# kotaro-kinoshita/yomitoku

Hardware: AMD Instinct MI355X
Metric: pages/sec (DocumentAnalyzer @1600x1200, lite model set) (higher is better)
Workload: dtype f32 held as two scaled fp16 planes per operand on the MFMA pipe: 3 x v_mfma_f32_32x32x16_f16 per product tile (products to 2^-21, below the fp32 accumulation's own rounding), fp32 accumulate, fp32 activations in HBM; attention, LayerNorm, the fused greedy step and every grid-starved launch exact fp3

## Files before the change

### yomitoku_amd/csrc/ymk_api.cpp

```cpp
#include "../../include/ymk.h"
#include "ymk_common.h"
#include "ymk_decstep.h"
#include "ymk_det.h"
#include "ymk_entry.h"
#include "ymk_seq.h"

struct ymk_model {
  ymk::Model* impl = nullptr;
  int device = 0;
};

#include <dlfcn.h>
namespace {
struct Roctx {
  int (*push)(const char*) = nullptr;
  int (*pop)() = nullptr;
  Roctx() {
    const char* on = std::getenv("YMK_ROCTX");
    if (on == nullptr || on[0] == '\0' || on[0] == '0') return;
    for (const char* name : {"librocprofiler-sdk-roctx.so", "libroctx64.so"}) {
      if (void* h = dlopen(name, RTLD_NOW | RTLD_GLOBAL)) {
        push = reinterpret_cast<int (*)(const char*)>(dlsym(h, "roctxRangePushA"));
        pop = reinterpret_cast<int (*)()>(dlsym(h, "roctxRangePop"));
        if (push && pop) return;
// ... 26 lines not shown
    return 1;                                       \
  }                                                 \
  catch (...) {                                     \
    ymk::set_error("unknown C++ exception");        \
    return 2;                                       \
  }

extern "C" {

int ymk_version(void) { return 100; }

const char* ymk_last_error(void) { return ymk::last_error().c_str(); }

int ymk_device_count(void) {
  int n = 0;
  if (hipGetDeviceCount(&n) != hipSuccess) return -1;
  return n;
}

ymk_model* ymk_model_create(const char* kind, int device) {
  try {
    YMK_CHECK(kind != nullptr, "kind is null");
    YMK_HIP(hipSetDevice(device));
    std::string k(kind);
    ymk::Model* impl = nullptr;
    if (k == "dbnet") impl = ymk::create_dbnet();
    else if (k == "parseq") impl = ymk::create_parseq();
    else if (k == "rtdetr") impl = ymk::create_rtdetr();
    else throw ymk::Error("unknown model kind: " + k);
    auto* m = new ymk_model();
    m->impl = impl;
    m->device = device;
    return m;
  } catch (const std::exception& e) {
    ymk::set_error(e.what());
    return nullptr;
  }
}

void ymk_model_destroy(ymk_model* m) {
  if (!m) return;
  (void)hipSetDevice(m->device);
  delete m->impl;
  delete m;
}

int ymk_model_set_param(ymk_model* m, const char* key, double value) {
  YMK_API_BEGIN
  YMK_CHECK(m && key, "null argument");
  const std::string k(key);
  if (k == "workspace_reuse") {
    YMK_CHECK(value == 0.0 || value == 1.0 || value == -1.0, "workspace_reuse must be 0 or 1 (-1: follow the process-wide default)");
    YMK_CHECK(!ymk::in_forward(), "workspace_reuse cannot change inside a forward");
  }
  m->impl->params[key] = value;
  if (m->impl->finalized && (k == "conv_split" || k == "conv_split_encoder")) {
    YMK_HIP(hipSetDevice(m->device));
    m->impl->prebuild_split();
  }
  YMK_API_END
}

int ymk_model_set_tensor(ymk_model* m, const char* name, const float* host_data, int ndim, const int64_t* dims) {
  YMK_API_BEGIN
  YMK_CHECK(m && name && host_data && (ndim == 0 || dims), "null argument");
  YMK_CHECK(!m->impl->finalized, "model already finalized");
  m->impl->ws.put(name, host_data, ndim, dims);
  YMK_API_END
}

int ymk_model_finalize(ymk_model* m) {
  YMK_API_BEGIN
  RoctxRange roctx_range("ymk_model_finalize");
  YMK_CHECK(m, "null model");
  YMK_HIP(hipSetDevice(m->device));
  m->impl->finalize();
  m->impl->prebuild_split();
  if (!ymk::debug_hazard_no_finalize_sync()) YMK_HIP(hipDeviceSynchronize());
  YMK_API_END
}

int ymk_model_reserve(ymk_model* m, int n, int h, int w, void* stream) {
  YMK_API_BEGIN
  RoctxRange roctx_range("ymk_model_reserve");
  YMK_CHECK(m && m->impl, "null argument");
  YMK_HIP(hipSetDevice(m->device));
  m->impl->reserve(n, h, w, (hipStream_t)stream);
  YMK_API_END
}

int64_t ymk_model_weight_bytes(const ymk_model* m) { return m ? (int64_t)m->impl->pool.bytes() : -1; }
int64_t ymk_model_workspace_bytes(const ymk_model* m) { return m ? (int64_t)m->impl->arena.capacity() : -1; }

int ymk_dbnet_forward(ymk_model* m, const float* x_dev, int n, int h, int w, float* prob_dev, void* stream) {
  YMK_API_BEGIN
  RoctxRange roctx_range("ymk_dbnet_forward");
  YMK_CHECK(m && x_dev && prob_dev, "null argument");
  YMK_HIP(hipSetDevice(m->device));
  ymk::dbnet_forward(m->impl, x_dev, n, h, w, prob_dev, (hipStream_t)stream);
  YMK_API_END
}

int ymk_parseq_dims(ymk_model* m, int* num_steps, int* num_classes) {
  YMK_API_BEGIN
  YMK_CHECK(m && num_steps && num_classes, "null argument");
  ymk::parseq_dims(m->impl, num_steps, num_classes);
  YMK_API_END
}

int ymk_parseq_forward(ymk_model* m, const float* x_dev, int b, int w, float* logits_dev, int* out_len, int* ar_steps,
                       void* stream) {
  YMK_API_BEGIN
  RoctxRange roctx_range("ymk_parseq_forward");
  YMK_CHECK(m && x_dev && logits_dev && out_len && ar_steps, "null argument");
  YMK_HIP(hipSetDevice(m->device));
  ymk::parseq_forward(m->impl, x_dev, b, w, logits_dev, out_len, ar_steps, (hipStream_t)stream);
  YMK_API_END
}

int ymk_parseq_forward_groups(ymk_model* m, const float* const* x_dev, const int* b, const int* w, int n_groups,
                              float* logits_dev, int* out_len, int* ar_steps, void* stream) {
  YMK_API_BEGIN
  RoctxRange roctx_range("ymk_parseq_forward_groups");
  YMK_CHECK(m && x_dev && b && w && logits_dev && out_len && ar_steps, "null argument");
  YMK_HIP(hipSetDevice(m->device));
  ymk::parseq_forward_groups(m->impl, x_dev, b, w, n_groups, logits_dev, out_len, ar_steps, (hipStream_t)stream);
  YMK_API_END
}

int ymk_parseq_token_stats(const float* logits_dev, int rows, int num_classes, int* ids_dev, float* probs_dev,
                           void* stream) {
  YMK_API_BEGIN
  RoctxRange roctx_range("ymk_parseq_token_stats");
  YMK_CHECK(logits_dev && ids_dev && probs_dev, "null argument");
  ymk::row_maxprob((hipStream_t)stream, logits_dev, rows, num_classes, ids_dev, probs_dev);
  YMK_API_END
}

int ymk_rtdetr_forward(ymk_model* m, const float* x_dev, int b, int h, int w, float* logits_dev, float* boxes_dev,
                       void* stream) {
  YMK_API_BEGIN
  RoctxRange roctx_range("ymk_rtdetr_forward");
  YMK_CHECK(m && x_dev && logits_dev && boxes_dev, "null argument");
  YMK_HIP(hipSetDevice(m->device));
  ymk::rtdetr_forward(m->impl, x_dev, b, h, w, logits_dev, boxes_dev, (hipStream_t)stream);
  YMK_API_END
}

int ymk_debug_option(const char* key, int value) {
  YMK_API_BEGIN
  YMK_CHECK(key != nullptr, "null key");
  const std::string k(key);
  YMK_CHECK(ymk::conv_debug_option(k, value) || ymk::parseq_debug_option(k, value) || ymk::decstep_debug_option(k, value) ||
                ymk::conv_split_debug_option(k, value) || ymk::runtime_debug_option(k, value),
            "unknown debug option: " + k);
  YMK_API_END
}

int ymk_stat(const char* key, int64_t* value) {
  YMK_API_BEGIN
  YMK_CHECK(key != nullptr && value != nullptr, "null argument");
  long long v = 0;
  YMK_CHECK(ymk::conv_split_stat(std::string(key), &v) || ymk::runtime_stat(std::string(key), &v) || ymk::parseq_stat(std::string(key), &v), std::string("unknown counter: ") + key);
  *value = v;
  YMK_API_END
}

int ymk_amax_check_counters(int64_t* out4) {
  YMK_API_BEGIN
  YMK_CHECK(out4 != nullptr, "null argument");
  long long v[4];
  ymk::amax_check_counters(v);
  for (int i = 0; i < 4; ++i) out4[i] = v[i];
  YMK_API_END
}

int ymk_prof_begin(void) {
  YMK_API_BEGIN
  ymk::prof_begin();
  YMK_API_END
}

int ymk_prof_end(double* conv_ms, double* conv_flop, int64_t* conv_launches) {
  YMK_API_BEGIN
  YMK_CHECK(conv_ms && conv_flop && conv_launches, "null argument");
  ymk::prof_end(conv_ms, conv_flop, conv_launches);
  YMK_API_END
}

int ymk_prof_bytes(double* conv_bytes) {
  YMK_API_BEGIN
  YMK_CHECK(conv_bytes, "null argument");
  *conv_bytes = ymk::prof_bytes();
  YMK_API_END
}

int ymk_prof_launch_table(double* ms, double* flop, double* bytes, double* mfma_products, int64_t capacity, int64_t* count) {
  YMK_API_BEGIN
  YMK_CHECK(count != nullptr && capacity >= 0 && (capacity == 0 || (ms && flop && bytes && mfma_products)), "null argument");
  *count = ymk::prof_launch_table(ms, flop, bytes, mfma_products, capacity);
  YMK_API_END
}

int ymk_op_plan_workspace(int64_t n, const int64_t* sizes, const int64_t* release_pos, int64_t* offsets_out, int64_t* peak_out,
                          int64_t* live_bound_out) {
  YMK_API_BEGIN
  YMK_CHECK(n >= 0 && (n == 0 || (sizes && offsets_out)), "plan_workspace: bad argument");
  std::vector<size_t> sz((size_t)n), off((size_t)n);
  for (int64_t k = 0; k < n; ++k) {
    YMK_CHECK(sizes[k] >= 0, "plan_workspace: negative size");
    sz[(size_t)k] = (size_t)sizes[k];
  }
  size_t peak = 0, live = 0;
  ymk::plan_workspace((size_t)n, sz.data(), release_pos, off.data(), &peak, &live);
  for (int64_t k = 0; k < n; ++k) offsets_out[k] = (int64_t)off[(size_t)k];
  if (peak_out) *peak_out = (int64_t)peak;
  if (live_bound_out) *live_bound_out = (int64_t)live;
  YMK_API_END
}

int ymk_op_conv2d(const float* x_dev, int n, int h, int w, int c, const float* w_host_oihw, int cout, int cin, int kh,
                  int kw, const float* scale_host, const float* bias_host, const float* res_dev, int stride, int pad,
                  int dil, int act, int tap4, float* y_dev, void* stream) {
  YMK_API_BEGIN
  using namespace ymk;
  DevicePool pool;
  ConvW cw;
  cw.cout = cout;
  cw.cin = tap4 ? 4 : cin;
  cw.kh = kh;
  cw.kw = kw;
  cw.mode = tap4 ? 1 : 0;
  std::vector<float> panel;
  pack_conv_weight(w_host_oihw, cout, cin, kh, kw, tap4 != 0, panel, cw.kpad, cw.ctiles);
  cw.w = pool.upload(panel);
  if (scale_host) cw.scale = pool.upload(scale_host, cout);
  if (bias_host) cw.bias = pool.upload(bias_host, cout);
  Tensor in{const_cast<float*>(x_dev), n, h, w, c, c};
  const int oh = conv_out_dim(h, kh, stride, pad, dil), ow = conv_out_dim(w, kw, stride, pad, dil);
  Tensor out{y_dev, n, oh, ow, cout, cout};
  Tensor res{const_cast<float*>(res_dev), n, oh, ow, cout, cout};
  ConvArgs a;
  a.stride = stride;
  a.pad = pad;
  a.dil = dil;
  a.act = act;
  a.res = res_dev ? &res : nullptr;
  SplitCtxOwner split_ctx;
  ConvSplitScope scope(-1, split_ctx.get(), 0);
  conv2d((hipStream_t)stream, in, cw, a, out);
  YMK_HIP(hipStreamSynchronize((hipStream_t)stream));
  YMK_API_END
}

static ymk::ConvW op_conv_weight(ymk::DevicePool& pool, const float* w_host_oihw, int cout, int cin, int kh, int kw, bool tap4,
                                 const float* scale_host, const float* bias_host) {
  using namespace ymk;
  ConvW cw;
  cw.cout = cout;
  cw.cin = tap4 ? 4 : cin;
  cw.kh = kh;
  cw.kw = kw;
  cw.mode = tap4 ? 1 : 0;
  std::vector<float> panel;
  pack_conv_weight(w_host_oihw, cout, cin, kh, kw, tap4, panel, cw.kpad, cw.ctiles);
  cw.w = pool.upload(panel);
  std::vector<float> scale, bias;
  if (scale_host) scale.assign(scale_host, scale_host + cout);
  if (bias_host) bias.assign(bias_host, bias_host + cout);
  if (scale_host) cw.scale = pool.upload(scale);
  if (bias_host) cw.bias = pool.upload(bias);
  plane_bound(cw, w_host_oihw, (size_t)cin * kh * kw, scale, bias);
  return cw;
}

int ymk_op_conv2d_view(const float* x_dev, int n, int h, int w, int c, int in_ld, const float* w_host_oihw, int cout, int kh, int kw,
                       int tap4, const float* scale_host, const float* bias_host, const float* res_dev, int res_ld, int res_post,
                       int stride_h, int stride_w, int pad, int dil, int act, const int* row_group_dev, const int* group_open_dev,
                       const unsigned* amax_in_dev, unsigned* amax_out_dev, float* y_dev, int out_ld, void* stream) {
  YMK_API_BEGIN
  using namespace ymk;
  YMK_CHECK(x_dev && w_host_oihw && y_dev, "null argument");
  YMK_CHECK(n > 0 && h > 0 && w > 0 && c > 0 && in_ld > 0 && cout > 0 && kh > 0 && kw > 0 && res_ld >= 0 && out_ld > 0 &&
                stride_h > 0 && stride_w > 0 && pad >= 0 && dil > 0,
            "conv2d_view: sizes, strides and leading dimensions are positive (res_ld may be 0)");
  hipStream_t s = (hipStream_t)stream;
  DevicePool pool;
  const ConvW cw = op_conv_weight(pool, w_host_oihw, cout, c, kh, kw, tap4 != 0, scale_host, bias_host);
  SplitCtxOwner split_ctx;
  ConvSplitScope scope(-1, split_ctx.get(), 0);
  if (row_group_dev || group_open_dev) {
    YMK_CHECK(kh == 1 && kw == 1 && stride_h == 1 && stride_w == 1 && pad == 0 && !res_post && !tap4,
              "conv2d_view: a row predicate comes with a plain linear layer");
    gemm(s, x_dev, n * h * w, c, in_ld, cw, act, res_dev, res_ld, y_dev, out_ld, row_group_dev, group_open_dev, EPI_STORE, amax_in_dev,
         amax_out_dev);
  } else {
    Tensor in{const_cast<float*>(x_dev), n, h, w, c, in_ld};
    const int oh = conv_out_dim(h, kh, stride_h, pad, dil), ow = conv_out_dim(w, kw, stride_w, pad, dil);
    Tensor out{y_dev, n, oh, ow, cout, out_ld};
    Tensor res{const_cast<float*>(res_dev), n, oh, ow, cout, res_ld};
    ConvArgs a;
    a.stride = stride_h;
    a.stride_w = stride_w;
    a.pad = pad;
    a.dil = dil;
    a.act = act;
    a.res = res_dev ? &res : nullptr;
    a.res_post = res_post != 0;
    a.amax_in = amax_in_dev;
    a.amax_out = amax_out_dev;
    conv2d(s, in, cw, a, out);
  }
  YMK_HIP(hipStreamSynchronize(s));
  YMK_API_END
}

// ... 475 lines not shown
```

### yomitoku_amd/csrc/ymk_seq.h

```cpp
#pragma once
#include "ymk_common.h"

namespace ymk {

void layernorm(hipStream_t s, const float* x, int ldx, int in_rows_mod, const float* g, const float* b, float eps,
               float* y, int ldy, int M, int D);
void add_pos_embed(hipStream_t s, float* x, const float* pos, int B, int gh, int gw, int full_gw, int D);

struct SeqTab {
  const int *qoff = nullptr, *qlen = nullptr, *koff = nullptr, *klen = nullptr;
};

void flash_attention(hipStream_t s, const float* q, const float* k, const float* v, float* o, int B, int H, int Lq, int Lk,
                     int hd, int ldq, int ldk, int ldv, int ldo, long bsq, long bsk, long bsv, long bso, float scale,
                     const SeqTab* tab = nullptr, const unsigned* amax_q = nullptr, const unsigned* amax_k = nullptr,
                     const unsigned* amax_v = nullptr);
void small_attention(hipStream_t s, const float* q, const float* k, const float* v, float* o, int B, int H, int Lq, int Lk,
                     int hd, int ldq, int ldk, int ldv, int ldo, long bsq, long bsk, long bsv, long bso, float scale,
                     const unsigned char* mask_qk, int ld_mask, const unsigned char* kpm, int ld_kpm,
                     const SeqTab* tab = nullptr);
void nar_cross_attention(hipStream_t s, const float* q, const float* k, const float* v, float* o, int B, int H, int Lq, int Lk,
                         int hd, int ldq, int ldk, int ldv, int ldo, long bsk, long bsv, long bso, float scale,
                         const SeqTab* tab = nullptr);
void init_decode(hipStream_t s, int* tok, int ld_tok, int* state, int bos_id, int pad_id, int B);

void ctx_embed_ln(hipStream_t s, const int* tok, int ld_tok, int pos0, int npos, const float* emb, const float* posq,
                  const float* g, const float* be, float eps, float* out, int out_rows, int D, int B);
void greedy_step(hipStream_t s, const float* logits, long ld_b, int C, int step, int num_steps, int* tok, int* raw,
                 int ld_tok, int* state, int eos_id, int rep_on, int period_max, int min_run_p1, int min_repeats,
                 int* not_done, const int* prev_not_done, int* arrived, int* host_flag, int B, const int* gid = nullptr,
                 int* gopen = nullptr, int ng = 1, int partials = 0);
void publish_open(hipStream_t s, const int* not_done, const int* prev_not_done, int* host_flag);
void refine_prep(hipStream_t s, const int* raw, int ld_tok, int S, int bos_id, int eos_id, int* tok2, unsigned char* kpm,
                 int B, const int* gid = nullptr, const int* gsteps = nullptr);
void row_argmax(hipStream_t s, const float* logits, int rows, int C, int* out);
void rep_cut(hipStream_t s, float* logits, long ld_b, int C, int S, const int* state, int eos_id, int B);
void row_maxprob(hipStream_t s, const float* logits, int rows, int C, int* ids, float* probs);
void tile_rows(hipStream_t s, const float* src, int rows, int D, float* dst, int B);
void fill_i32(hipStream_t s, int* p, int v, size_t n);

}
```

### yomitoku_amd/csrc/ymk_seq.hip

```cpp
#include "ymk_common.h"
#include "ymk_f16_planes.h"
#include "ymk_seq.h"

namespace ymk {


__device__ __forceinline__ float wave_sum(float v) {
#pragma unroll
  for (int o = 32; o > 0; o >>= 1) v += __shfl_xor(v, o, 64);
  return v;
}
__device__ __forceinline__ float wave_max(float v) {
#pragma unroll
  for (int o = 32; o > 0; o >>= 1) v = fmaxf(v, __shfl_xor(v, o, 64));
  return v;
}

__global__ void k_layernorm(const float* __restrict__ x, int ldx, int in_rows_mod, const float* __restrict__ g,
                            const float* __restrict__ b, float eps, float* __restrict__ y, int ldy, int M, int D) {
  const int row = blockIdx.x * (blockDim.x >> 6) + (threadIdx.x >> 6);
  const int lane = threadIdx.x & 63;
  if (row >= M) return;
  const float* xr = x + (size_t)(in_rows_mod > 0 ? row % in_rows_mod : row) * ldx;
  float4 v[4];
  const int nv = D >> 2;
  float s = 0.f;
#pragma unroll
  for (int i = 0; i < 4; ++i) {
    const int c = lane + 64 * i;
    if (c < nv) {
      v[i] = *reinterpret_cast<const float4*>(xr + c * 4);
      s += (v[i].x + v[i].y) + (v[i].z + v[i].w);
    }
  }
  const float mean = wave_sum(s) / (float)D;
  float q = 0.f;
#pragma unroll
  for (int i = 0; i < 4; ++i) {
    const int c = lane + 64 * i;
    if (c < nv) {
      const float a = v[i].x - mean, bb = v[i].y - mean, cc = v[i].z - mean, d = v[i].w - mean;
      q += (a * a + bb * bb) + (cc * cc + d * d);
    }
  }
  const float rstd = 1.f / sqrtf(wave_sum(q) / (float)D + eps);
#pragma unroll
  for (int i = 0; i < 4; ++i) {
    const int c = lane + 64 * i;
    if (c < nv) {
      const float4 gg = *reinterpret_cast<const float4*>(g + c * 4);
      const float4 be = *reinterpret_cast<const float4*>(b + c * 4);
      float4 o;
      o.x = (v[i].x - mean) * rstd * gg.x + be.x;
      o.y = (v[i].y - mean) * rstd * gg.y + be.y;
      o.z = (v[i].z - mean) * rstd * gg.z + be.z;
      o.w = (v[i].w - mean) * rstd * gg.w + be.w;
      *reinterpret_cast<float4*>(y + (size_t)row * ldy + c * 4) = o;
    }
  }
}
void layernorm(hipStream_t s, const float* x, int ldx, int in_rows_mod, const float* g, const float* b, float eps,
               float* y, int ldy, int M, int D) {
  YMK_CHECK(D % 4 == 0 && D <= 1024, "layernorm: D must be a multiple of 4, <= 1024");
  if (M == 0) return;
  hipLaunchKernelGGL(k_layernorm, dim3((M + 3) / 4), dim3(256), 0, s, x, ldx, in_rows_mod, g, b, eps, y, ldy, M, D);
  YMK_HIP(hipGetLastError());
}

__global__ void k_add_pos(float* __restrict__ x, const float* __restrict__ pos, int gh, int gw, int full_gw, int D4,
                          size_t total) {
  for (size_t i = (size_t)blockIdx.x * blockDim.x + threadIdx.x; i < total; i += (size_t)gridDim.x * blockDim.x) {
    const int c4 = (int)(i % D4);
    const size_t tok = i / D4;
    const int cc = (int)(tok % gw);
    const int rr = (int)((tok / gw) % gh);
    float4 v = reinterpret_cast<float4*>(x)[i];
    const float4 p = reinterpret_cast<const float4*>(pos)[(size_t)(rr * full_gw + cc) * D4 + c4];
    v.x += p.x; v.y += p.y; v.z += p.z; v.w += p.w;
    reinterpret_cast<float4*>(x)[i] = v;
  }
}
void add_pos_embed(hipStream_t s, float* x, const float* pos, int B, int gh, int gw, int full_gw, int D) {
  const size_t total = (size_t)B * gh * gw * (D / 4);
  size_t g = (total + 255) / 256;
  if (g > 4096) g = 4096;
  hipLaunchKernelGGL(k_add_pos, dim3((int)g), dim3(256), 0, s, x, pos, gh, gw, full_gw, D / 4, total);
  YMK_HIP(hipGetLastError());
}

struct AttnP {
  const float *q, *k, *v;
  float* o;
  int ldq, ldk, ldv, ldo;
  long bsq, bsk, bsv, bso;
  int Lq, Lk, H;
  float scale;
  const int *qoff, *qlen, *koff, *klen;
  const unsigned *amax_q, *amax_k, *amax_v;
};

template <int HD, int HDR = HD>
__global__ __launch_bounds__(256, 1) void k_flash_attn(AttnP p) {
  constexpr int KT = 64;
  constexpr int LDH = HD + 4;
  constexpr int NKC = HDR / 8;
  constexpr int NDC = HD / 32;
  constexpr int LPT = (KT * HDR / 4) / 256;
  static_assert(HD % 32 == 0 && HDR % 8 == 0 && HDR <= HD && (KT * HDR / 4) % 256 == 0, "head dim");
  __shared__ __attribute__((aligned(16))) float lds[2 * 2 * KT * LDH];

  const int t = threadIdx.x, wv = t >> 6, lane = t & 63, li = lane & 31, lh = lane >> 5;
  const int b = blockIdx.z, h = blockIdx.y;
  const int q0 = blockIdx.x * 128 + wv * 32;
  const float* qb = p.q + (size_t)b * p.bsq + h * HDR;
  const float* kb = p.k + (size_t)b * p.bsk + h * HDR;
  const float* vb = p.v + (size_t)b * p.bsv + h * HDR;
  float* ob = p.o + (size_t)b * p.bso + h * HDR;
  int Lq = p.Lq, Lk = p.Lk;
  if (p.koff) {
    const size_t r = (size_t)p.koff[b];
    kb = p.k + r * p.ldk + h * HDR;
    vb = p.v + r * p.ldv + h * HDR;
    Lk = p.klen[b];
  }
  if (p.qoff) {
    const size_t r = (size_t)p.qoff[b];
    qb = p.q + r * p.ldq + h * HDR;
    ob = p.o + r * p.ldo + h * HDR;
    Lq = p.qlen[b];
  }
  if ((int)blockIdx.x * 128 >= Lq) return;

  f32x4 qf[NKC];
  {
    const int qi = min(q0 + li, Lq - 1);
    const float* qr = qb + (size_t)qi * p.ldq;
#pragma unroll
    for (int kc = 0; kc < NKC; ++kc) {
      qf[kc] = *reinterpret_cast<const f32x4*>(qr + kc * 8 + lh * 4);
      qf[kc] *= p.scale;
    }
  }

  f32x16 oacc[NDC];
#pragma unroll
  for (int dc = 0; dc < NDC; ++dc)
#pragma unroll
    for (int r = 0; r < 16; ++r) oacc[dc][r] = 0.f;
  float m_run = -INFINITY, l_run = 0.f;

  f32x4 rk[LPT], rv[LPT];
  auto load_kv = [&](int k0) {
// ... 173 lines not shown
      const int idx = t + 256 * i;
      const int row = idx / (HDR / 4), c4 = idx - row * (HDR / 4);
      *reinterpret_cast<f32x4*>(Ks + row * LDH + c4 * 4) = rk[i];
      *reinterpret_cast<f32x4*>(Vs + row * LDH + c4 * 4) = rv[i];
    }
  };

  const int ntiles = (Lk + KT - 1) / KT;
  load_kv(0);
  store_kv(0);
  __syncthreads();
  for (int tt = 0; tt < ntiles; ++tt) {
    const int buf = tt & 1;
    if (tt + 1 < ntiles) load_kv((tt + 1) * KT);
    const float* Ks = lds + buf * (2 * KT * LDH);
    const float* Vs = Ks + KT * LDH;
#pragma unroll
    for (int sub = 0; sub < (q0 < Lq ? KT / 32 : 0); ++sub) {
      const int kbase = tt * KT + sub * 32;
      if (kbase >= Lk) break;
      f32x16 sacc;
#pragma unroll
      for (int r = 0; r < 16; ++r) sacc[r] = 0.f;
      const float* kr = Ks + (sub * 32 + li) * LDH + lh * 8;
#pragma unroll
      for (int ks = 0; ks < NKS; ++ks) {
        const f32x4 a = *reinterpret_cast<const f32x4*>(kr + ks * 16);
        const f32x4 c = *reinterpret_cast<const f32x4*>(kr + ks * 16 + 4);
        const float x[8] = {a.x, a.y, a.z, a.w, c.x, c.y, c.z, c.w};
        f16x8 kh, kl;
        f16_split8(x, s_k, kh, kl);
        sacc = __builtin_amdgcn_mfma_f32_32x32x16_f16(kl, qh[ks], sacc, 0, 0, 0);
        sacc = __builtin_amdgcn_mfma_f32_32x32x16_f16(kh, ql[ks], sacc, 0, 0, 0);
        sacc = __builtin_amdgcn_mfma_f32_32x32x16_f16(kh, qh[ks], sacc, 0, 0, 0);
      }
      float mt = -INFINITY;
#pragma unroll
      for (int r = 0; r < 16; ++r) {
        const int key = kbase + (r & 3) + 8 * (r >> 2) + 4 * lh;
        sacc[r] = key >= Lk ? -INFINITY : sacc[r] * s_unscale;
        mt = fmaxf(mt, sacc[r]);
      }
      mt = fmaxf(mt, __shfl_xor(mt, 32, 64));
      const float m_new = fmaxf(m_run, mt);
      const float alpha = __expf(m_run - m_new);
      float ps = 0.f;
#pragma unroll
      for (int r = 0; r < 16; ++r) {
        sacc[r] = __expf(sacc[r] - m_new);
        ps += sacc[r];
      }
      ps += __shfl_xor(ps, 32, 64);
      l_run = l_run * alpha + ps;
      m_run = m_new;
      f16x8 ph[2], pl[2];
#pragma unroll
      for (int j = 0; j < 2; ++j) {
        const float x[8] = {sacc[8 * j], sacc[8 * j + 1], sacc[8 * j + 2], sacc[8 * j + 3], sacc[8 * j + 4], sacc[8 * j + 5], sacc[8 * j + 6], sacc[8 * j + 7]};
        f16_split8(x, 16384.f, ph[j], pl[j]);
      }
#pragma unroll
      for (int dc = 0; dc < NDC; ++dc) {
#pragma unroll
        for (int r = 0; r < 16; ++r) oacc[dc][r] *= alpha;
        const float* vr = Vs + (sub * 32 + 4 * lh) * LDH + dc * 32 + li;
#pragma unroll
        for (int j = 0; j < 2; ++j) {
          float x[8];
#pragma unroll
          for (int e = 0; e < 8; ++e) {
            const int r = 8 * j + e;
            x[e] = vr[((r & 3) + 8 * (r >> 2)) * LDH];
          }
          f16x8 vh, vl;
          f16_split8(x, s_v, vh, vl);
          oacc[dc] = __builtin_amdgcn_mfma_f32_32x32x16_f16(vl, ph[j], oacc[dc], 0, 0, 0);
          oacc[dc] = __builtin_amdgcn_mfma_f32_32x32x16_f16(vh, pl[j], oacc[dc], 0, 0, 0);
          oacc[dc] = __builtin_amdgcn_mfma_f32_32x32x16_f16(vh, ph[j], oacc[dc], 0, 0, 0);
        }
      }
    }
    if (tt + 1 < ntiles) store_kv(buf ^ 1);
    __syncthreads();
  }
  const int qi = q0 + li;
  if (qi < Lq) {
    const float inv = o_unscale / l_run;
    float* orow = ob + (size_t)qi * p.ldo;
#pragma unroll
    for (int dc = 0; dc < NDC; ++dc)
#pragma unroll
      for (int g = 0; g < 4; ++g) {
        f32x4 w;
        w.x = oacc[dc][4 * g + 0] * inv;
        w.y = oacc[dc][4 * g + 1] * inv;
        w.z = oacc[dc][4 * g + 2] * inv;
        w.w = oacc[dc][4 * g + 3] * inv;
        if (dc * 32 + 8 * g + 4 * lh < HDR) *reinterpret_cast<f32x4*>(orow + dc * 32 + 8 * g + 4 * lh) = w;
      }
  }
}

void flash_attention(hipStream_t s, const float* q, const float* k, const float* v, float* o, int B, int H, int Lq, int Lk,
                     int hd, int ldq, int ldk, int ldv, int ldo, long bsq, long bsk, long bsv, long bso, float scale,
                     const SeqTab* tab, const unsigned* amax_q, const unsigned* amax_k, const unsigned* amax_v) {
  if (B == 0 || Lq == 0) return;
  YMK_CHECK(Lk > 0, "attention: no keys");
  YMK_CHECK(ldq % 4 == 0 && ldk % 4 == 0 && ldv % 4 == 0 && ldo % 4 == 0, "attention: strides must be multiples of 4");
  AttnP p{q, k, v, o, ldq, ldk, ldv, ldo, bsq, bsk, bsv, bso, Lq, Lk, H, scale, nullptr, nullptr, nullptr, nullptr, amax_q, amax_k, amax_v};
  if (tab) {
    p.qoff = tab->qoff;
    p.qlen = tab->qlen;
    p.koff = tab->koff;
    p.klen = tab->klen;
    YMK_CHECK((p.qoff == nullptr) == (p.qlen == nullptr) && (p.koff == nullptr) == (p.klen == nullptr), "attention: offset and length tables come in pairs");
  }
  dim3 grid((Lq + 127) / 128, H, B);
  const bool f16 = amax_q && amax_k && amax_v && scale <= 1.f && scale > 0.f && conv_effective_split() == SPLIT_F16X2 && ldq % 4 == 0;
  if (f16 && (hd == 32 || hd == 64 || hd == 96 || hd == 48)) {
    if (hd == 32) hipLaunchKernelGGL(k_flash_attn_f16<32>, grid, dim3(256), 0, s, p);
    else if (hd == 64) hipLaunchKernelGGL(k_flash_attn_f16<64>, grid, dim3(256), 0, s, p);
    else if (hd == 96) hipLaunchKernelGGL(k_flash_attn_f16<96>, grid, dim3(256), 0, s, p);
    else hipLaunchKernelGGL((k_flash_attn_f16<64, 48>), grid, dim3(256), 0, s, p);
    YMK_HIP(hipGetLastError());
    return;
  }
  if (hd == 32) hipLaunchKernelGGL(k_flash_attn<32>, grid, dim3(256), 0, s, p);
  else if (hd == 64) hipLaunchKernelGGL(k_flash_attn<64>, grid, dim3(256), 0, s, p);
  else if (hd == 96) hipLaunchKernelGGL(k_flash_attn<96>, grid, dim3(256), 0, s, p);
  else if (hd == 48) hipLaunchKernelGGL((k_flash_attn<64, 48>), grid, dim3(256), 0, s, p);
  else {
    YMK_CHECK(Lk <= 1024 && hd <= 128, "attention: head dim " + std::to_string(hd) + " is only supported for <= 1024 keys per sample");
    small_attention(s, q, k, v, o, B, H, Lq, Lk, hd, ldq, ldk, ldv, ldo, bsq, bsk, bsv, bso, scale, nullptr, 0, nullptr, 0, tab);
    return;
  }
  YMK_HIP(hipGetLastError());
}

struct SmallAttnP {
  const float *q, *k, *v;
  float* o;
  int ldq, ldk, ldv, ldo;
  long bsq, bsk, bsv, bso;
  int Lq, Lk, H, hd;
  float scale;
  const unsigned char* mask_qk;
  int ld_mask;
  const unsigned char* kpm;
  int ld_kpm;
  const int *koff, *klen;
  const int *qoff, *qlen;
  int vec4;
};
__global__ __launch_bounds__(64) void k_small_attn(SmallAttnP p) {
  __shared__ float prob[1024];
  __shared__ float qs[128];
  const int lane = threadIdx.x;
  const int qi = blockIdx.x, h = blockIdx.y, b = blockIdx.z;
  if (p.qoff && qi >= p.qlen[b]) return;
  const size_t qrow0 = p.qoff ? (size_t)p.qoff[b] : 0;
  const float* qr = (p.qoff ? p.q + qrow0 * p.ldq : p.q + (size_t)b * p.bsq) + (size_t)qi * p.ldq + h * p.hd;
  for (int d = lane; d < p.hd; d += 64) qs[d] = qr[d] * p.scale;
  __syncthreads();
  const float* kb = p.k + (size_t)b * p.bsk + h * p.hd;
  const float* vb = p.v + (size_t)b * p.bsv + h * p.hd;
  int Lk = p.Lk;
  if (p.koff) {
    kb = p.k + (size_t)p.koff[b] * p.ldk + h * p.hd;
    vb = p.v + (size_t)p.koff[b] * p.ldv + h * p.hd;
    Lk = p.klen[b];
  }
  float mx = -INFINITY;
  for (int k = lane; k < Lk; k += 64) {
    bool blocked = false;
    if (p.mask_qk) blocked = p.mask_qk[(size_t)qi * p.ld_mask + k] != 0;
    if (p.kpm) blocked = blocked || p.kpm[(size_t)b * p.ld_kpm + k] != 0;
    float sc = -INFINITY;
    if (!blocked) {
      const float* kr = kb + (size_t)k * p.ldk;
      float a = 0.f;
      if (p.vec4) {
        for (int d = 0; d < p.hd; d += 4) {
          const float4 kk = *reinterpret_cast<const float4*>(kr + d);
          a += qs[d] * kk.x + qs[d + 1] * kk.y + qs[d + 2] * kk.z + qs[d + 3] * kk.w;
        }
      } else {
        for (int d = 0; d < p.hd; ++d) a += qs[d] * kr[d];
      }
      sc = a;
    }
    prob[k] = sc;
    mx = fmaxf(mx, sc);
  }
  mx = wave_max(mx);
  float sum = 0.f;
  for (int k = lane; k < Lk; k += 64) {
    const float e = __expf(prob[k] - mx);
    prob[k] = e;
    sum += e;
  }
  sum = wave_sum(sum);
  __syncthreads();
  const float inv = 1.f / sum;
  float* orow = (p.qoff ? p.o + qrow0 * p.ldo : p.o + (size_t)b * p.bso) + (size_t)qi * p.ldo + h * p.hd;
  for (int d = lane; d < p.hd; d += 64) {
    float a = 0.f;
    for (int k = 0; k < Lk; ++k) a += prob[k] * vb[(size_t)k * p.ldv + d];
    orow[d] = a * inv;
  }
}
void small_attention(hipStream_t s, const float* q, const float* k, const float* v, float* o, int B, int H, int Lq, int Lk,
                     int hd, int ldq, int ldk, int ldv, int ldo, long bsq, long bsk, long bsv, long bso, float scale,
                     const unsigned char* mask_qk, int ld_mask, const unsigned char* kpm, int ld_kpm, const SeqTab* tab) {
  if (B == 0 || Lq == 0) return;
  YMK_CHECK(Lk > 0 && Lk <= 1024 && hd <= 128, "small attention: Lk <= 1024, hd <= 128");
  const int vec4 = hd % 4 == 0 && ldk % 4 == 0 && bsk % 4 == 0 && ((uintptr_t)k & 15) == 0;
  SmallAttnP p{q, k, v, o, ldq, ldk, ldv, ldo, bsq, bsk, bsv, bso, Lq, Lk, H, hd, scale, mask_qk, ld_mask, kpm, ld_kpm,
               tab ? tab->koff : nullptr, tab ? tab->klen : nullptr, tab ? tab->qoff : nullptr, tab ? tab->qlen : nullptr, vec4};
  YMK_CHECK(!tab || (!mask_qk && !kpm), "small attention: ragged batches come without masks");
  hipLaunchKernelGGL(k_small_attn, dim3(Lq, H, B), dim3(64), 0, s, p);
  YMK_HIP(hipGetLastError());
}

__global__ void k_ctx_embed_ln(const int* __restrict__ tok, int ld_tok, int pos0, int npos, const float* __restrict__ emb,
                               const float* __restrict__ posq, const float* __restrict__ g, const float* __restrict__ be,
                               float eps, float sqrt_d, float* __restrict__ out, int out_rows, int D, int B) {
  const int w = blockIdx.x * (blockDim.x >> 6) + (threadIdx.x >> 6);
  const int lane = threadIdx.x & 63;
  if (w >= B * npos) return;
  const int b = w / npos, pos = pos0 + (w - b * npos);
  const int token = tok[(size_t)b * ld_tok + pos];
  const float* er = emb + (size_t)token * D;
  const float* pr = pos > 0 ? posq + (size_t)(pos - 1) * D : nullptr;
  float v[16];
  float s = 0.f;
  const int per = (D + 63) / 64;
  for (int i = 0; i < per; ++i) {
    const int c = lane + 64 * i;
    float x = 0.f;
    if (c < D) {
      x = sqrt_d * er[c];
      if (pr) x = pr[c] + x;
      s += x;
    }
    v[i] = x;
  }
  const float mean = wave_sum(s) / (float)D;
  float q = 0.f;
  for (int i = 0; i < per; ++i) {
    const int c = lane + 64 * i;
    if (c < D) q += (v[i] - mean) * (v[i] - mean);
  }
  const float rstd = 1.f / sqrtf(wave_sum(q) / (float)D + eps);
  float* orow = out + ((size_t)b * out_rows + pos) * D;
  for (int i = 0; i < per; ++i) {
    const int c = lane + 64 * i;
    if (c < D) orow[c] = (v[i] - mean) * rstd * g[c] + be[c];
  }
}
void ctx_embed_ln(hipStream_t s, const int* tok, int ld_tok, int pos0, int npos, const float* emb, const float* posq,
                  const float* g, const float* be, float eps, float* out, int out_rows, int D, int B) {
  YMK_CHECK(D <= 1024, "ctx_embed: D <= 1024");
  const int waves = B * npos;
  if (waves == 0) return;
  hipLaunchKernelGGL(k_ctx_embed_ln, dim3((waves + 3) / 4), dim3(256), 0, s, tok, ld_tok, pos0, npos, emb, posq, g, be, eps,
                     sqrtf((float)D), out, out_rows, D, B);
  YMK_HIP(hipGetLastError());
}

constexpr int ROW_RV = 32;
template <bool WITH_SUM>
__device__ __forceinline__ void row_reduce_256(const float* __restrict__ row, int C, float* sv, int* si, float& mx, int& am,
                                               float& sum) {
  const int t = threadIdx.x;
  float best = -INFINITY;
  int bi = t < C ? t : 0x7fffffff;
  float v[ROW_RV];
  const bool in_regs = C <= 256 * ROW_RV;
  if (in_regs) {
#pragma unroll
    for (int i = 0; i < ROW_RV; ++i) {
      const int c = t + 256 * i;
      v[i] = c < C ? row[c] : -INFINITY;
    }
#pragma unroll
    for (int i = 0; i < ROW_RV; ++i)
      if (v[i] > best) {
        best = v[i];
        bi = t + 256 * i;
      }
  } else {
    for (int c = t; c < C; c += 256) {
      const float x = row[c];
      if (x > best) {
        best = x;
        bi = c;
      }
    }
  }
  sv[t] = best;
  si[t] = bi;
  __syncthreads();
  for (int o = 128; o > 0; o >>= 1) {
    if (t < o) {
      const float v2 = sv[t + o];
      const int i2 = si[t + o];
      if (v2 > sv[t] || (v2 == sv[t] && i2 < si[t])) {
        sv[t] = v2;
        si[t] = i2;
      }
    }
    __syncthreads();
  }
  mx = sv[0];
  am = si[0];
  if (WITH_SUM) {
    __syncthreads();
    float acc = 0.f;
    if (in_regs) {
#pragma unroll
      for (int i = 0; i < ROW_RV; ++i)
        if (t + 256 * i < C) acc += expf(v[i] - mx);
    } else {
      for (int c = t; c < C; c += 256) acc += expf(row[c] - mx);
    }
    sv[t] = acc;
    __syncthreads();
    for (int o = 128; o > 0; o >>= 1) {
      if (t < o) sv[t] += sv[t + o];
      __syncthreads();
    }
    sum = sv[0];
  }
}

__global__ __launch_bounds__(256) void k_greedy_step(const float* __restrict__ logits, long ld_b, int C, int step,
                                                     int num_steps, int* __restrict__ tok, int* __restrict__ raw,
                                                     int ld_tok, int* __restrict__ state, int eos_id, int rep_on,
                                                     int period_max, int min_run_p1, int min_repeats,
                                                     int* __restrict__ not_done, const int* __restrict__ prev_not_done,
                                                     int* __restrict__ arrived, int* __restrict__ host_flag,
                                                     const int* __restrict__ gid, int* __restrict__ gopen, int ng, int partials,
                                                     int flags) {
  const int b = blockIdx.x, t = threadIdx.x;
  if (prev_not_done && *prev_not_done == 0) return;
  const int g = gid ? gid[b] : 0;
  const bool frozen = gid && step > 0 && gopen[(size_t)(step - 1) * ng + g] == 0;
  __shared__ float sv[256];
  __shared__ int si[256];
  if (!frozen && !partials) {
    float mx, unused;
    int am;
    row_reduce_256<false>(logits + (size_t)b * ld_b, C, sv, si, mx, am, unused);
  }
  if (!frozen && partials) {
    const float2* pr = reinterpret_cast<const float2*>(logits + (size_t)b * ld_b);
    float v = -INFINITY;
    int i = 0x7fffffff;
    if (t < C) {
      const float2 q = pr[t];
      v = q.x;
      i = __float_as_int(q.y);
    }
    sv[t] = v;
    si[t] = i;
    __syncthreads();
    for (int o = 128; o > 0; o >>= 1) {
      if (t < o) {
        const float v2 = sv[t + o];
        const int i2 = si[t + o];
        if (v2 > sv[t] || (v2 == sv[t] && i2 < si[t])) {
          sv[t] = v2;
          si[t] = i2;
// ... 199 lines not shown
```

Measured before the change: 133.4.

## Add per-head small attention kernel reusing K/V across query rows

Adds a new small-attention kernel that launches one block per (head, batch), stages V in shared memory and K in registers once, and has four waves sweep the query rows while prefetching the next rows' queries and masks. This removes the repeated K/V reloads that the old one-block-per-query kernel did for every query row. It is on by default for hd 32/64, Lk<=128 and Lq>=8, with a debug option and a launch counter. The dot-product accumulation order is pinned to keep results matching the old kernel. The cost is fewer blocks and serial row processing per block, which can limit parallelism when B*H is small.

```diff
diff --git a/yomitoku_amd/csrc/ymk_api.cpp b/yomitoku_amd/csrc/ymk_api.cpp
--- a/yomitoku_amd/csrc/ymk_api.cpp
+++ b/yomitoku_amd/csrc/ymk_api.cpp
@@ -202,7 +202,7 @@
   YMK_CHECK(key != nullptr, "null key");
   const std::string k(key);
   YMK_CHECK(ymk::conv_debug_option(k, value) || ymk::parseq_debug_option(k, value) || ymk::decstep_debug_option(k, value) ||
-                ymk::conv_split_debug_option(k, value) || ymk::runtime_debug_option(k, value),
+                ymk::conv_split_debug_option(k, value) || ymk::seq_debug_option(k, value) || ymk::runtime_debug_option(k, value),
             "unknown debug option: " + k);
   YMK_API_END
 }
@@ -211,7 +211,9 @@
   YMK_API_BEGIN
   YMK_CHECK(key != nullptr && value != nullptr, "null argument");
   long long v = 0;
-  YMK_CHECK(ymk::conv_split_stat(std::string(key), &v) || ymk::runtime_stat(std::string(key), &v) || ymk::parseq_stat(std::string(key), &v), std::string("unknown counter: ") + key);
+  YMK_CHECK(ymk::conv_split_stat(std::string(key), &v) || ymk::runtime_stat(std::string(key), &v) || ymk::parseq_stat(std::string(key), &v) ||
+                ymk::seq_stat(std::string(key), &v),
+            std::string("unknown counter: ") + key);
   *value = v;
   YMK_API_END
 }
diff --git a/yomitoku_amd/csrc/ymk_seq.h b/yomitoku_amd/csrc/ymk_seq.h
--- a/yomitoku_amd/csrc/ymk_seq.h
+++ b/yomitoku_amd/csrc/ymk_seq.h
@@ -19,6 +19,8 @@
                      int hd, int ldq, int ldk, int ldv, int ldo, long bsq, long bsk, long bsv, long bso, float scale,
                      const unsigned char* mask_qk, int ld_mask, const unsigned char* kpm, int ld_kpm,
                      const SeqTab* tab = nullptr);
+bool seq_debug_option(const std::string& key, int value);
+bool seq_stat(const std::string& key, long long* value);
 void nar_cross_attention(hipStream_t s, const float* q, const float* k, const float* v, float* o, int B, int H, int Lq, int Lk,
                          int hd, int ldq, int ldk, int ldv, int ldo, long bsk, long bsv, long bso, float scale,
                          const SeqTab* tab = nullptr);
diff --git a/yomitoku_amd/csrc/ymk_seq.hip b/yomitoku_amd/csrc/ymk_seq.hip
--- a/yomitoku_amd/csrc/ymk_seq.hip
+++ b/yomitoku_amd/csrc/ymk_seq.hip
@@ -1,3 +1,5 @@
+#include <atomic>
+
 #include "ymk_common.h"
 #include "ymk_f16_planes.h"
 #include "ymk_seq.h"
@@ -477,9 +479,15 @@
   const int *qoff, *qlen;
   int vec4;
 };
+__device__ __forceinline__ float small_attn_dot4(float a, const float4 q4, const float4 kk) {
+#pragma clang fp contract(off)
+  const float g = q4.x * kk.x + q4.y * kk.y + q4.z * kk.z + q4.w * kk.w;
+  return a + g;
+}
+__device__ __forceinline__ float small_attn_pv(float a, float pk, float vk) { return fmaf(pk, vk, a); }
 __global__ __launch_bounds__(64) void k_small_attn(SmallAttnP p) {
   __shared__ float prob[1024];
-  __shared__ float qs[128];
+  __shared__ __align__(16) float qs[128];
   const int lane = threadIdx.x;
   const int qi = blockIdx.x, h = blockIdx.y, b = blockIdx.z;
   if (p.qoff && qi >= p.qlen[b]) return;
@@ -507,7 +515,7 @@
       if (p.vec4) {
         for (int d = 0; d < p.hd; d += 4) {
           const float4 kk = *reinterpret_cast<const float4*>(kr + d);
-          a += qs[d] * kk.x + qs[d + 1] * kk.y + qs[d + 2] * kk.z + qs[d + 3] * kk.w;
+          a = small_attn_dot4(a, *reinterpret_cast<const float4*>(qs + d), kk);
         }
       } else {
         for (int d = 0; d < p.hd; ++d) a += qs[d] * kr[d];
@@ -530,10 +538,153 @@
   float* orow = (p.qoff ? p.o + qrow0 * p.ldo : p.o + (size_t)b * p.bso) + (size_t)qi * p.ldo + h * p.hd;
   for (int d = lane; d < p.hd; d += 64) {
     float a = 0.f;
-    for (int k = 0; k < Lk; ++k) a += prob[k] * vb[(size_t)k * p.ldv + d];
+    for (int k = 0; k < Lk; ++k) a = small_attn_pv(a, prob[k], vb[(size_t)k * p.ldv + d]);
     orow[d] = a * inv;
   }
 }
+
+constexpr int SA_ROWS_WAVES = 4;
+__device__ __forceinline__ void wave_lds_sync() {
+  __builtin_amdgcn_fence(__ATOMIC_RELEASE, "wavefront");
+  __builtin_amdgcn_wave_barrier();
+  __builtin_amdgcn_fence(__ATOMIC_ACQUIRE, "wavefront");
+}
+template <int HD, int KPL>
+__global__ __launch_bounds__(SA_ROWS_WAVES * 64) void k_small_attn_rows(SmallAttnP p) {
+  constexpr int QW = 64 / HD, LKP = 64 * KPL, NT = SA_ROWS_WAVES * 64;
+  __shared__ __align__(16) float vs[LKP * HD];
+  __shared__ __align__(16) float prob[SA_ROWS_WAVES][QW][LKP];
+  __shared__ __align__(16) float qs[SA_ROWS_WAVES][QW][HD];
+  __shared__ unsigned char kblk[LKP];
+  const int tid = threadIdx.x, lane = tid & 63, wave = tid >> 6;
+  const int h = blockIdx.x, b = blockIdx.y;
+  const int Lk = p.Lk;
+  const float* kb = p.k + (size_t)b * p.bsk + h * HD;
+  const float* vb = p.v + (size_t)b * p.bsv + h * HD;
+  for (int i = tid; i < Lk * (HD / 4); i += NT) {
+    const int k = i / (HD / 4), c = i - k * (HD / 4);
+    reinterpret_cast<float4*>(vs)[i] = *reinterpret_cast<const float4*>(vb + (size_t)k * p.ldv + 4 * c);
+  }
+  for (int k = tid; k < Lk; k += NT) kblk[k] = p.kpm ? p.kpm[(size_t)b * p.ld_kpm + k] : (unsigned char)0;
+  float4 kreg[KPL][HD / 4];
+#pragma unroll
+  for (int j = 0; j < KPL; ++j) {
+    const int k = lane + 64 * j;
+    const float* kr = kb + (size_t)(k < Lk ? k : 0) * p.ldk;
+#pragma unroll
+    for (int c = 0; c < HD / 4; ++c) kreg[j][c] = k < Lk ? *reinterpret_cast<const float4*>(kr + 4 * c) : make_float4(0.f, 0.f, 0.f, 0.f);
+  }
+  __syncthreads();
+  const int g_pv = lane / HD, d_pv = lane - g_pv * HD;
+  auto fetch = [&](int q0, float (&qn)[QW], unsigned char (&mn)[QW][KPL]) {
+#pragma unroll
+    for (int g = 0; g < QW; ++g) {
+      const int qi = q0 + g;
+      qn[g] = 0.f;
+#pragma unroll
+      for (int j = 0; j < KPL; ++j) mn[g][j] = 0;
+      if (qi >= p.Lq) continue;
+      if (lane < HD) qn[g] = (p.q + (size_t)b * p.bsq + (size_t)qi * p.ldq + h * HD)[lane];
+#pragma unroll
+      for (int j = 0; j < KPL; ++j) {
+        const int k = lane + 64 * j;
+        if (p.mask_qk && k < Lk) mn[g][j] = p.mask_qk[(size_t)qi * p.ld_mask + k];
+      }
+    }
+  };
+  float qc[QW];
+  unsigned char mc[QW][KPL];
+  fetch(wave * QW, qc, mc);
+  for (int q0 = wave * QW; q0 < p.Lq; q0 += SA_ROWS_WAVES * QW) {
+    float qn[QW];
+    unsigned char mn[QW][KPL];
+    fetch(q0 + SA_ROWS_WAVES * QW, qn, mn);
+    float inv[QW];
+#pragma unroll
+    for (int g = 0; g < QW; ++g) {
+      inv[g] = 0.f;
+      const int qi = q0 + g;
+      if (qi >= p.Lq) continue;
+      if (lane < HD) qs[wave][g][lane] = qc[g] * p.scale;
+      wave_lds_sync();
+      float4 qv[HD / 4];
+#pragma unroll
+      for (int c = 0; c < HD / 4; ++c) qv[c] = *reinterpret_cast<const float4*>(&qs[wave][g][4 * c]);
+      float sc[KPL];
+      float mx = -INFINITY;
+#pragma unroll
+      for (int j = 0; j < KPL; ++j) {
+        const int k = lane + 64 * j;
+        sc[j] = -INFINITY;
+        if (k < Lk) {
+          const bool blocked = mc[g][j] != 0 || kblk[k] != 0;
+          if (!blocked) {
+            float a = 0.f;
+#pragma unroll
+            for (int c = 0; c < HD / 4; ++c) a = small_attn_dot4(a, qv[c], kreg[j][c]);
+            sc[j] = a;
+          }
+          mx = fmaxf(mx, sc[j]);
+        }
+      }
+      mx = wave_max(mx);
+      float sum = 0.f;
+#pragma unroll
+      for (int j = 0; j < KPL; ++j) {
+        const int k = lane + 64 * j;
+        if (k < Lk) {
+          const float e = __expf(sc[j] - mx);
+          prob[wave][g][k] = e;
+          sum += e;
+        }
+      }
+      sum = wave_sum(sum);
+      inv[g] = 1.f / sum;
+    }
+    wave_lds_sync();
+    if (q0 + g_pv < p.Lq) {
+      const float* pr = prob[wave][g_pv];
+      const float* vc = vs + d_pv;
+      float a = 0.f;
+      int k = 0;
+      for (; k + 4 <= Lk; k += 4) {
+        const float4 p4 = *reinterpret_cast<const float4*>(pr + k);
+        a = small_attn_pv(a, p4.x, vc[(k + 0) * HD]);
+        a = small_attn_pv(a, p4.y, vc[(k + 1) * HD]);
+        a = small_attn_pv(a, p4.z, vc[(k + 2) * HD]);
+        a = small_attn_pv(a, p4.w, vc[(k + 3) * HD]);
+      }
+      for (; k < Lk; ++k) a = small_attn_pv(a, pr[k], vc[k * HD]);
+      float iv = inv[0];
+#pragma unroll
+      for (int g = 1; g < QW; ++g) iv = g_pv == g ? inv[g] : iv;
+      float* orow = p.o + (size_t)b * p.bso + (size_t)(q0 + g_pv) * p.ldo + h * HD;
+      orow[d_pv] = a * iv;
+    }
+    wave_lds_sync();
+#pragma unroll
+    for (int g = 0; g < QW; ++g) {
+      qc[g] = qn[g];
+#pragma unroll
+      for (int j = 0; j < KPL; ++j) mc[g][j] = mn[g][j];
+    }
+  }
+}
+
+static std::atomic<int> g_small_attn_rows{1};
+static std::atomic<long long> g_small_attn_rows_launches{0};
+bool seq_debug_option(const std::string& key, int value) {
+  if (key != "small_attn_rows") return false;
+  g_small_attn_rows = value;
+  return true;
+}
+bool seq_stat(const std::string& key, long long* value) {
+  if (key != "small_attn_rows_launches") return false;
+  *value = g_small_attn_rows_launches.load();
+  return true;
+}
+constexpr int SMALL_ATTN_ROWS_MIN_LQ = 8;
+
 void small_attention(hipStream_t s, const float* q, const float* k, const float* v, float* o, int B, int H, int Lq, int Lk,
                      int hd, int ldq, int ldk, int ldv, int ldo, long bsq, long bsk, long bsv, long bso, float scale,
                      const unsigned char* mask_qk, int ld_mask, const unsigned char* kpm, int ld_kpm, const SeqTab* tab) {
@@ -543,7 +694,18 @@
   SmallAttnP p{q, k, v, o, ldq, ldk, ldv, ldo, bsq, bsk, bsv, bso, Lq, Lk, H, hd, scale, mask_qk, ld_mask, kpm, ld_kpm,
                tab ? tab->koff : nullptr, tab ? tab->klen : nullptr, tab ? tab->qoff : nullptr, tab ? tab->qlen : nullptr, vec4};
   YMK_CHECK(!tab || (!mask_qk && !kpm), "small attention: ragged batches come without masks");
-  hipLaunchKernelGGL(k_small_attn, dim3(Lq, H, B), dim3(64), 0, s, p);
+  const int rows_mode = g_small_attn_rows.load(std::memory_order_relaxed);
+  const bool rows = rows_mode != 0 && !tab && Lq >= (rows_mode == 2 ? 2 : SMALL_ATTN_ROWS_MIN_LQ) && (hd == 32 || hd == 64) && Lk <= 128 &&
+                    vec4 && ldv % 4 == 0 && bsv % 4 == 0 && ((uintptr_t)v & 15) == 0 && B <= 65535;
+  if (rows) {
+    const dim3 grid(H, B), block(SA_ROWS_WAVES * 64);
+    if (hd == 32 && Lk <= 64) hipLaunchKernelGGL((k_small_attn_rows<32, 1>), grid, block, 0, s, p);
+    else if (hd == 32) hipLaunchKernelGGL((k_small_attn_rows<32, 2>), grid, block, 0, s, p);
+    else if (Lk <= 64) hipLaunchKernelGGL((k_small_attn_rows<64, 1>), grid, block, 0, s, p);
+    else hipLaunchKernelGGL((k_small_attn_rows<64, 2>), grid, block, 0, s, p);
+    ++g_small_attn_rows_launches;
+  } else
+    hipLaunchKernelGGL(k_small_attn, dim3(Lq, H, B), dim3(64), 0, s, p);
   YMK_HIP(hipGetLastError());
 }
 
```

Measured after the change: 130.1. 0.975x the previous value.
